# joncampbell123/composite-video-simulator

Hardware: AMD Instinct MI355X
Metric: frames/sec (output frames = fields; 720x486 NTSC, preset '-vhs'; steady-state pipelined throughput, 4 steps in flight) (higher is better)
Workload: dtype f64; 1 GPU; 720x486 30fps 10s colour-bars clip, preset '-vhs': 300 frames -> 600 fields per GPU per step, frame-round-robin over 1 GPU(s); steps_in_flight=4, mode=exact (bit-identical to the reference: fp64, no FMA contraction)

## Files before the change

composite-video-simulator_amd/csrc/ntsc_decode_fast.hip:

```cpp
#pragma clang fp contract(off)

namespace ntscsim {
namespace fastdec {

typedef uint32_t v4u __attribute__((ext_vector_type(4)));
#ifdef NTSC_PLAIN_OUT_STORES
#define NTSC_OUT_STORE(p, v) (*(p) = (v))
#else
#define NTSC_OUT_STORE(p, v) __builtin_nontemporal_store((v), (p))
#endif
typedef __attribute__((address_space(1))) v4u *g_v4u_ptr;
typedef __attribute__((address_space(1))) const v4u *g_cv4u_ptr;
DEV v4u to_v4u(const uint4 &a) { return v4u{a.x, a.y, a.z, a.w}; }
typedef __attribute__((address_space(1))) uint32_t *g_u32_ptr;
typedef __attribute__((address_space(1))) const uint32_t *g_cu32_ptr;

#ifdef NTSC_NO_STEP_SCHED_BARRIER
#define NTSC_STEP_SCHED_BARRIER() ((void)0)
#else
#define NTSC_STEP_SCHED_BARRIER() __builtin_amdgcn_sched_barrier(0)
#endif

struct LaneRand32 {
    uint32_t p3, p2, p1;
    int pos;
    DEV void init(uint32_t *ring, const uint32_t *state, int stride, int lane, int o)
    {
        for (int j = 0; j < 31; j++) {
            const uint32_t w = state[(size_t)j * stride];
            const int sl = (o + j) & 31;
            ring[sl * 64 + lane] = w;
            if (sl == 0) ring[32 * 64 + lane] = w;
            if (j == 28) p3 = w;
            if (j == 29) p2 = w;
            if (j == 30) p1 = w;
        }
        pos = (o + 31) & 31;
    }
    DEV uint32_t next(uint32_t *ring, int lane)
    {
        const uint32_t v = ring[(pos + 1) * 64 + lane] + p3;
        ring[pos * 64 + lane] = v;
        if (pos == 0) ring[32 * 64 + lane] = v;
        p3 = p2; p2 = p1; p1 = v;
        pos = (pos + 1) & 31;
        return v >> 1;
    }
    template <int K>
    DEV uint32_t draw(uint32_t *rb, bool first_slot_is_zero)
    {
        const uint32_t v = rb[(K + 1) * 64] + p3;
        rb[K * 64] = v;
        if (K == 0 && first_slot_is_zero) rb[32 * 64] = v;
        p3 = p2; p2 = p1; p1 = v;
        return v >> 1;
    }
};

template <class RT>
struct Casc3;
template <>
struct Casc3<double> {
    double r0, r1, r2;
    DEV void reset(double v, double a) { const double r = v - (v * a); r0 = r1 = r2 = r; }
    DEV double push(double s, double a, double &m2)
    {
        const double p0 = (s * a) + r0;
        const double m0 = p0 * a;
        r0 = p0 - m0;
        const double p1 = m0 + r1;
        const double m1 = p1 * a;
        r1 = p1 - m1;
        const double p2 = m1 + r2;
        m2 = p2 * a;
        r2 = p2 - m2;
        return p2;
    }
    DEV double push(double s, double a) { double m; return push(s, a, m); }
};
template <>
struct Casc3<float> {
    float p0, p1, p2;
    DEV void reset(float v, float) { p0 = p1 = p2 = v; }
    DEV float push(float s, float a, float &m2)
    {
        p0 = __builtin_fmaf(a, s - p0, p0);
        p1 = __builtin_fmaf(a, p0 - p1, p1);
        p2 = __builtin_fmaf(a, p1 - p2, p2);
        m2 = 0.f;
        return p2;
    }
    DEV float push(float s, float a) { float m; return push(s, a, m); }
};
template <class RT>
struct PoleHp;
template <>
struct PoleHp<double> {
    double r;
    DEV void reset(double v, double a) { r = v - (v * a); }
    DEV double hp(double s, double s_times_a, double a)
    {
        const double p = s_times_a + r;
        r = p - (p * a);
        return s - p;
    }
};
template <>
struct PoleHp<float> {
    float p;
    DEV void reset(float v, float) { p = v; }
    DEV float hp(float s, float, float a) { p = __builtin_fmaf(a, s - p, p); return s - p; }
};

DEV int sdiv4s(int n) { return (n + (int)((unsigned)n >> 30)) >> 2; }

DEV int scale_back50(int c, unsigned mul, unsigned shift)
{
    const int sg = c >> 31;
    const unsigned a = (unsigned)((c ^ sg) - sg) * 50u;
    const int q = (int)(__umulhi(a, mul) >> shift);
    return (q ^ sg) - sg;
}

struct DemodR {
    int c0, c1, c2, csum;
    int w0, w1, w2, w3, w4, w5;
    int y0, y1, y2, y3, y4;
    int ieP, qeP, ieN, qeN;
    DEV void init()
    {
        c0 = c1 = c2 = csum = 0;
        w0 = w1 = w2 = w3 = w4 = w5 = 0;
        y0 = y1 = y2 = y3 = y4 = 0;
        ieP = qeP = ieN = qeN = 0;
    }
    template <bool ODD, int NEG, bool LUMA, bool BK = false>
    DEV void push(int ct, bool hi, int sneg, int &Yo, int &Io, int &Qo, unsigned bmul = 0, unsigned bshift = 0)
    {
        const int yb = sdiv4s(csum + ct);
        int ch = ct - yb;
        if (BK) ch = scale_back50(ch, bmul, bshift);
        csum = csum - c0 + ct;
        c0 = c1; c1 = c2; c2 = ct;
        w0 = w1; w1 = w2; w2 = w3; w3 = w4; w4 = w5; w5 = ch;
        if (LUMA) { Yo = y0; y0 = y1; y1 = y2; y2 = y3; y3 = y4; y4 = yb; }
        if (ODD) {
            const int a = hi ? w3 : w1, b = hi ? w4 : w2;
            if (NEG == 0) { ieN = a; qeN = b; }
            else if (NEG == 1) { ieN = -a; qeN = -b; }
            else { ieN = (a ^ sneg) - sneg; qeN = (b ^ sneg) - sneg; }
            Io = (ieP + ieN) >> 1;
            Qo = (qeP + qeN) >> 1;
        } else {
            Io = ieN; Qo = qeN;
            ieP = ieN; qeP = qeN;
        }
    }
    template <bool BK = false, bool ANY = false>
    DEV void push_edge(int ct, int t, unsigned xi, bool hi, int W, int xe, int &Yo, int &Io, int &Qo,
                       unsigned bmul = 0, unsigned bshift = 0)
    {
        const int yb = sdiv4(c0 + c1 + c2 + ct);
        int ch = ct - yb;
        if (BK) ch = scale_back50(ch, bmul, bshift);
        csum = c1 + c2 + ct;
        c0 = c1; c1 = c2; c2 = ct;
        w0 = w1; w1 = w2; w2 = w3; w3 = w4; w4 = w5; w5 = ch;
        Yo = y0; y0 = y1; y1 = y2; y2 = y3; y3 = y4; y4 = yb;
        const int x = t - 7;
        int I, Q;
        if (x & 1) {
            const bool m = (x + 1 + (int)xi + 1) < W;
            const bool od = ANY && (xi & 1u) != 0;
            const int a = hi ? (od ? w4 : w3) : (od ? w2 : w1), b = hi ? (od ? w5 : w4) : (od ? w3 : w2);
            const bool pos = ANY ? ((((x + 1 + 2 * (int)xi) & 2) != 0) && !(xi == 1u && x == -1)) : ((x & 3) == 1);
            ieN = m ? (pos ? a : -a) : 0;
            qeN = m ? (pos ? b : -b) : 0;
            I = (ieP + ieN) >> 1;
            Q = (qeP + qeN) >> 1;
        } else {
            I = ieN; Q = qeN;
            ieP = ieN; qeP = qeN;
        }
        if (x >= xe) { I = 0; Q = 0; }
        Io = I; Qo = Q;
    }
};

struct DemodS {
    int c1, pA, pB;
    int e1, e2, o1, o2;
    int y0, y1, y2, y3, y4;
    int ieP, qeP, ieN, qeN;
    DEV void from(const DemodR &D, bool pick_next)
    {
        c1 = D.c2; pA = D.c2 + D.c1; pB = D.c1 + D.c0;
        if (pick_next) { e1 = D.w4; e2 = D.w2; o1 = D.w5; o2 = D.w3; }
        else           { e1 = D.w5; e2 = D.w3; o1 = D.w4; o2 = D.w2; }
        y0 = D.y0; y1 = D.y1; y2 = D.y2; y3 = D.y3; y4 = D.y4;
        ieP = D.ieP; qeP = D.qeP; ieN = D.ieN; qeN = D.qeN;
    }
    DEV void to(DemodR &D, bool pick_next) const
    {
        D.c2 = c1; D.c1 = pA - c1; D.c0 = pB - D.c1; D.csum = D.c0 + D.c1 + D.c2;
        D.w0 = 0; D.w1 = 0;
        if (pick_next) { D.w4 = e1; D.w2 = e2; D.w5 = o1; D.w3 = o2; }
        else           { D.w5 = e1; D.w3 = e2; D.w4 = o1; D.w2 = o2; }
        D.y0 = y0; D.y1 = y1; D.y2 = y2; D.y3 = y3; D.y4 = y4;
        D.ieP = ieP; D.qeP = qeP; D.ieN = ieN; D.qeN = qeN;
    }
    template <bool PICK, bool NEG, bool LUMA, bool BK = false, bool MASK = false, bool ANY = false>
    DEV void push(int ct, bool hi, int dm, int &Yo, int &Io, int &Qo, unsigned bmul = 0, unsigned bshift = 0,
                  bool odd = false, int mo = 0)
    {
        const int p = ct + c1;
        const int yb = sdiv4s(p + pB);
        int ch = ct - yb;
        if (BK) ch = scale_back50(ch, bmul, bshift);
        c1 = ct; pB = pA; pA = p;
        if (LUMA) { Yo = y0; y0 = y1; y1 = y2; y2 = y3; y3 = y4; y4 = yb; }
        if (PICK) {
            int a, b;
            if (ANY) {
                const int aL = odd ? o2 : e2, aH = odd ? o1 : e1;
                const int bL = odd ? e1 : o2, bH = odd ? ch : o1;
                a = hi ? aH : aL; b = hi ? bH : bL;
                const int sg = NEG ? ~mo : mo;
                a = (a ^ sg) - sg; b = (b ^ sg) - sg;
            } else {
                a = hi ? e1 : e2; b = hi ? o1 : o2;
                if (NEG) { a = -a; b = -b; }
            }
            e2 = e1; e1 = ch;
            if (MASK) { a &= dm; b &= dm; }
            ieN = a; qeN = b;
            Io = (ieP + ieN) >> 1;
            Qo = (qeP + qeN) >> 1;
        } else {
            o2 = o1; o1 = ch;
            Io = ieN; Qo = qeN;
            ieP = ieN; qeP = qeN;
        }
    }
};

template <bool VHS, class RT>
struct State {
    DemodR D1, D2;
    int l0, l1, l2, lsum;
    Casc3<RT> vl, vcU, vcV, sh, oU, oV;
    PoleHp<RT> vpre;
    int Yprev, Uraw, Vraw;
    RT Uf2[2];
    LaneRand32 rng;
    int nU, nV;
};

template <class RT, bool WR = false, bool BK = false, bool SV = false, bool XA = false, bool FO = false>
struct Const {
    static constexpr bool fullout = FO;
    static constexpr int SH = FO ? 3 : 0;
    RT a_oi, a_oq;
    uint32_t *xs;
    static constexpr bool wraps = WR;
    static constexpr bool back = BK;
    static constexpr bool svideo = SV;
    static constexpr bool anyxi = XA;
    bool odd;
    int mo;
    int ms[4];
    unsigned bmul, bshift;
    int wrapoff;
    int wrapA, wrapS;
    unsigned xi;
    bool hi;
    int W, xe, lane;
    int d, SKT, LOFF;
    int mL, mNL;
    int bA, bC;
    int dm;
    RT cosv, sinv;
    RT a_vc, a_vl, a_sh, a_tv, sharp2;
    int *tailU;
    size_t rstride;
    __amdgpu_buffer_rsrc_t comp;
    int vbase;
    int rowbytes;
};

#ifndef NTSC_COMP_LOAD2_AUX
#define NTSC_COMP_LOAD2_AUX 2
#endif
template <int AUX = 0, class CT>
DEV int cs_load(const CT &C, int x)
{
#ifdef NTSC_AB_NOLOAD
    return C.vbase + x;
#endif
    unsigned off = (unsigned)C.vbase + (unsigned)x * (unsigned)C.rowbytes;
    if constexpr (CT::wraps) off += (unsigned)((((C.wrapA - x) ^ C.wrapS) >> 31) & C.wrapoff);
    return __builtin_amdgcn_raw_buffer_load_b32(C.comp, (int)off, 0, AUX);
}

DEV int opaque_v(int v) { asm volatile("" : "+v"(v)); return v; }
DEV int opaque_s(int v) { return __builtin_amdgcn_readfirstlane(v); }

DEV int wave_up(int v) { return __builtin_amdgcn_update_dpp(0, v, 0x138, 0xf, 0xf, false); }

DEV uint32_t cvt_sat_u32(double x) { uint32_t r; asm("v_cvt_u32_f64 %0, %1" : "=v"(r) : "v"(x)); return r; }
DEV uint32_t cvt_sat_u32(float x) { uint32_t r; asm("v_cvt_u32_f32 %0, %1" : "=v"(r) : "v"(x)); return r; }
DEV uint32_t umin32(uint32_t a, uint32_t b) { return a < b ? a : b; }

template <class RT>
DEV uint32_t yiq_to_bgra(int Yo, RT fU, RT fV)
{
    const RT y = (RT)Yo;
#ifdef NTSC_OLD_CLAMP
    int r = (int)((y + (RT(0.956) * fU)) + (RT(0.621) * fV)) >> 8;
    int g = (int)((y + (RT(-0.272) * fU)) + (RT(-0.647) * fV)) >> 8;
    int b = (int)((y + (RT(-1.106) * fU)) + (RT(1.703) * fV)) >> 8;
    r = r < 0 ? 0 : (r > 255 ? 255 : r);
    g = g < 0 ? 0 : (g > 255 ? 255 : g);
    b = b < 0 ? 0 : (b > 255 ? 255 : b);
    return (((uint32_t)r << 16) | (uint32_t)b) | ((uint32_t)g << 8);
#else
    const uint32_t r = umin32(cvt_sat_u32((y + (RT(0.956) * fU)) + (RT(0.621) * fV)) >> 8, 255u);
    const uint32_t g = umin32(cvt_sat_u32((y + (RT(-0.272) * fU)) + (RT(-0.647) * fV)) >> 8, 255u);
    const uint32_t b = umin32(cvt_sat_u32((y + (RT(-1.106) * fU)) + (RT(1.703) * fV)) >> 8, 255u);
    return ((r << 16) | b) | (g << 8);
#endif
}

struct Steady {
    DemodS D1, D2;
    int lc1, lpA, lpB;
    uint32_t *rb;
    bool rb0;
    int yd[4];
    int ud[2];
};

template <int DPH, int J, class RT, class CT>
DEV int vcr_step(const DevParams &P, State<true, RT> &S, Steady &T, const CT &C,
                 int pc, int pl, int &Yv, int &Uv, int &Vv)
{
    constexpr bool pick1 = ((DPH + J) & 1) != 0;
    constexpr bool neg1 = ((DPH + J) & 3) == 3;
    int Yd, U, V;
    T.D1.template push<pick1, neg1, false, CT::back, false, CT::anyxi>(pc, C.hi, -1, Yd, U, V, C.bmul, C.bshift, C.odd, C.mo);
    U += S.nU; V += S.nV;
    S.nU = sdiv2(S.nU + (int)umod31(S.rng.template draw<2 * J>(T.rb, T.rb0), P.m_cnoise) - P.cnoise_k);
    S.nV = sdiv2(S.nV + (int)umod31(S.rng.template draw<2 * J + 1>(T.rb, T.rb0), P.m_cnoise) - P.cnoise_k);
    const RT u = (RT)U, v = (RT)V;
    const RT Ud = rtrunc<RT>((u * C.cosv) - (v * C.sinv));
    const RT Vd = rtrunc<RT>((u * C.sinv) + (v * C.cosv));
    const int fU = (int)S.vcU.push(Ud, C.a_vc);
    const int fV = (int)S.vcV.push(Vd, C.a_vc);
    const int lp = pl + T.lc1;
    const int yb = sdiv4s(lp + T.lpB);
    T.lc1 = pl; T.lpB = T.lpA; T.lpA = lp;
    RT m2;
    RT s = S.vl.push((RT)yb, C.a_vl, m2);
    s += S.vpre.hp(s, m2, C.a_vl) * RT(1.6);
    const RT s0 = rtrunc<RT>(s);
    const RT ts = S.sh.push(s0, C.a_sh);
    const int Y = (int)(s0 + ((s0 - ts) * C.sharp2));
    U = ((wave_up(fU) & C.bA) + fU + C.bC) >> C.bC;
    V = ((wave_up(fV) & C.bA) + fV + C.bC) >> C.bC;
    Yv = Y; Uv = U; Vv = V;
    constexpr int J2 = (J + CT::SH) & 3;
    if constexpr (CT::anyxi) {
        const int chroma = (J2 & 1) ? (C.odd ? U : V) : (C.odd ? V : U);
        const int mm = C.ms[J2];
        return Y + ((chroma ^ mm) - mm);
    }
    const int chroma = (J2 & 1) ? V : U;
    const int mm = (J2 & 2) ? C.mNL : C.mL;
    return Y + ((chroma ^ mm) - mm);
}

template <bool VHS, int DPH, int J, class RT, class CT>
DEV uint32_t step(const DevParams &P, State<VHS, RT> &S, Steady &T, const CT &C, int pc, int pl)
{
    int Y, U, V;
    constexpr bool pick3 = ((J + 1 + CT::SH) & 1) != 0;
    constexpr bool neg3 = ((J + 1 + CT::SH) & 3) == 3;
    if constexpr (!VHS) {
        T.D1.template push<pick3, neg3, true, CT::back, true, CT::anyxi>(pc, C.hi, C.dm, Y, U, V, C.bmul, C.bshift, C.odd, C.mo);
    } else {
        int Yv, Uv, Vv;
        const int c2 = vcr_step<DPH, J, RT, CT>(P, S, T, C, pc, pl, Yv, Uv, Vv);
        if constexpr (CT::svideo) {
            Y = Yv; U = Uv & C.dm; V = Vv & C.dm;
        } else {
            T.D2.template push<pick3, neg3, true, false, true, CT::anyxi>(c2, C.hi, C.dm, Y, U, V, 0, 0, C.odd, C.mo);
        }
    }
    if constexpr (CT::fullout) {
        const int fUn = (int)S.oU.push((RT)U, C.a_oi);
        const RT fVd = rtrunc<RT>(S.oV.push((RT)V, C.a_oq));
        const int Yo = T.yd[J];
        T.yd[J] = Y;
        const RT fUd = (RT)T.ud[J & 1];
        T.ud[J & 1] = fUn;
        return yiq_to_bgra<RT>(Yo, fUd, fVd);
    } else {
        const RT fUd = rtrunc<RT>(S.oU.push((RT)U, C.a_tv));
        const RT fVd = rtrunc<RT>(S.oV.push((RT)V, C.a_tv));
        const int Yo = S.Yprev;
        S.Yprev = Y;
        return yiq_to_bgra<RT>(Yo, fUd, fVd);
    }
}

template <class RT, class CT>
DEV int vcr_edge(const DevParams &P, State<true, RT> &S, const CT &C, uint32_t *ring, int t, int &Yv, int &Uv, int &Vv)
{
    const int W = C.W;
    const int pc = t < W ? cs_load(C, t) : 0;
    int Y, U, V;
    S.D1.template push_edge<CT::back, CT::anyxi>(pc, t, C.xi, C.hi, W, C.xe, Y, U, V, C.bmul, C.bshift);
    const int x1 = t - 7;
    const bool in1 = x1 >= 0 && x1 < W;
    int fU = 0, fV = 0;
    if (in1) {
        U += S.nU; V += S.nV;
        S.nU = sdiv2(S.nU + (int)umod31(S.rng.next(ring, C.lane), P.m_cnoise) - P.cnoise_k);
        S.nV = sdiv2(S.nV + (int)umod31(S.rng.next(ring, C.lane), P.m_cnoise) - P.cnoise_k);
        const RT u = (RT)U, v = (RT)V;
        U = (int)((u * C.cosv) - (v * C.sinv));
        V = (int)((u * C.sinv) + (v * C.cosv));
        fU = (int)S.vcU.push((RT)U, C.a_vc);
        fV = (int)S.vcV.push((RT)V, C.a_vc);
        if (x1 >= W - C.d) {
            C.tailU[(size_t)(x1 & 15) * C.rstride] = U;
            C.tailU[(size_t)(16 + (x1 & 15)) * C.rstride] = V;
        }
    }
    const int x2 = x1 - C.d;
    const int xl = t - C.LOFF;
    const int pl = (xl >= 0 && xl < W) ? cs_load(C, xl) : 0;
    const int yb = sdiv4(S.l0 + S.l1 + S.l2 + pl);
    S.lsum = S.l1 + S.l2 + pl;
    S.l0 = S.l1; S.l1 = S.l2; S.l2 = pl;
    const bool in2 = x2 >= 0 && x2 < W;
    if (in2) {
        if (x2 >= W - C.d) {
            fU = C.tailU[(size_t)(x2 & 15) * C.rstride];
            fV = C.tailU[(size_t)(16 + (x2 & 15)) * C.rstride];
        }
        RT m2;
        RT s = S.vl.push((RT)yb, C.a_vl, m2);
        s += S.vpre.hp(s, m2, C.a_vl) * RT(1.6);
        const RT s0 = rtrunc<RT>(s);
        const RT ts = S.sh.push(s0, C.a_sh);
        Y = (int)(s0 + ((s0 - ts) * C.sharp2));
    }
    U = ((wave_up(fU) & C.bA) + fU + C.bC) >> C.bC;
    V = ((wave_up(fV) & C.bA) + fV + C.bC) >> C.bC;
    int c2 = 0;
    Yv = 0; Uv = 0; Vv = 0;
    if (in2) {
        Yv = Y; Uv = U; Vv = V;
        const unsigned s = (C.xi + (unsigned)x2) & 3u;
        int chroma = (s & 1u) ? V : U;
        if (s & 2u) chroma = -chroma;
        c2 = Y + chroma;
    }
    return c2;
}

template <bool VHS, class RT, class CT>
DEV bool edge_step(const DevParams &P, State<VHS, RT> &S, const CT &C, uint32_t *ring, int t,
                   uint32_t &px, int &xo_out)
{
    const int W = C.W;
    int Y, U, V;
    int x3 = t - 7;
    if constexpr (VHS) {
        int Yv, Uv, Vv;
        const int c2 = vcr_edge<RT, CT>(P, S, C, ring, t, Yv, Uv, Vv);
        const int x2 = t - 7 - C.d;
        if constexpr (CT::svideo) {
            Y = Yv; U = Uv; V = Vv;
            x3 = x2;
        } else {
            S.D2.template push_edge<false, CT::anyxi>(c2, x2, C.xi, C.hi, W, C.xe, Y, U, V);
            x3 = x2 - 7;
        }
    } else {
        const int pc = t < W ? cs_load(C, t) : 0;
        S.D1.template push_edge<CT::back, CT::anyxi>(pc, t, C.xi, C.hi, W, C.xe, Y, U, V, C.bmul, C.bshift);
    }
    if constexpr (CT::fullout) {
        if (x3 < 0 || x3 >= W + 4) return false;
        const bool in3f = x3 < W;
        if (!in3f) { U = 0; V = 0; Y = 0; }
        U &= C.dm; V &= C.dm;
        RT fUn = 0, fVn = 0;
        if (in3f) {
            fUn = rtrunc<RT>(S.oU.push((RT)U, C.a_oi));
            fVn = rtrunc<RT>(S.oV.push((RT)V, C.a_oq));
        }
        const int k3 = x3 & 3;
        const int Yo4 = (int)C.xs[k3 * 64], Ur4 = (int)C.xs[(4 + k3) * 64], Vr4 = (int)C.xs[(8 + k3) * 64];
        C.xs[k3 * 64] = (uint32_t)Y; C.xs[(4 + k3) * 64] = (uint32_t)U; C.xs[(8 + k3) * 64] = (uint32_t)V;
        const RT Uf = S.Uf2[0];
        S.Uf2[0] = S.Uf2[1]; S.Uf2[1] = fUn;
        const int xof = x3 - 4;
        if (xof < 0) return false;
        const RT Uo = xof < W - 2 ? Uf : (RT)Ur4;
        const RT Vo = xof < W - 4 ? fVn : (RT)Vr4;
        px = yiq_to_bgra<RT>(Yo4, Uo, Vo);
        xo_out = xof;
        return true;
    }
    if (x3 < 0 || x3 > W) return false;
    const bool in3 = x3 < W;
    if (!in3) { U = 0; V = 0; Y = 0; }
    U &= C.dm; V &= C.dm;
    RT fUd = 0, fVd = 0;
    if (in3) {
        fUd = rtrunc<RT>(S.oU.push((RT)U, C.a_tv));
        fVd = rtrunc<RT>(S.oV.push((RT)V, C.a_tv));
    }
    const int xo = x3 - 1;
    const int Yo = S.Yprev;
    const int Ur = S.Uraw, Vr = S.Vraw;
    S.Yprev = Y; S.Uraw = U; S.Vraw = V;
    if (xo < 0) return false;
    if (xo >= W - 1) { fUd = (RT)Ur; fVd = (RT)Vr; }
    px = yiq_to_bgra<RT>(Yo, fUd, fVd);
    xo_out = xo;
    return true;
}

template <bool VHS, int DPH, class RT, class CT>
DEV int steady(const DevParams &P, State<VHS, RT> &S, const CT &C, uint32_t *ring, uint32_t *lring,
               uint32_t *ostage, const unsigned long long *orow, uint32_t *drow, bool is_out, int t)
{
    const int t_end = C.W - (C.d > 7 ? C.d - 7 : 0);
    const int SKT = C.SKT, LOFF = C.LOFF, lane = C.lane;
    if (t + 4 > t_end) return t;
    if (VHS && (S.rng.pos & 7)) return t;
    Steady T;
    constexpr bool pick3_next = ((1 + CT::SH) & 1) != 0;
    T.D1.from(S.D1, VHS ? (DPH & 1) != 0 : pick3_next);
    T.D2.from(S.D2, pick3_next);
    T.lc1 = S.l2; T.lpA = S.l2 + S.l1; T.lpB = S.l1 + S.l0;
    if constexpr (CT::fullout) {
#pragma unroll
        for (int q = 0; q < 4; q++) T.yd[q] = (int)C.xs[q * 64];
        T.ud[0] = (int)S.Uf2[0]; T.ud[1] = (int)S.Uf2[1];
    }
    DemodS &Dout = (VHS && !CT::svideo) ? T.D2 : T.D1;
    if (!(VHS && CT::svideo)) { Dout.ieP &= C.dm; Dout.qeP &= C.dm; Dout.ieN &= C.dm; Dout.qeN &= C.dm; }
    int sbase = VHS ? S.rng.pos : 0;
    constexpr int PD = 4;
    int pc[PD], pl[PD];
#pragma unroll
    for (int j = 0; j < PD; j++) { pc[j] = cs_load(C, t + j); pl[j] = VHS ? cs_load<NTSC_COMP_LOAD2_AUX>(C, t + j - LOFF) : 0; }
    constexpr bool PFTOP = !VHS;
    int pend_x = -1;
#ifdef NTSC_FAST_LANE_STORE
#define NTSC_FAST_FLUSH()                                                                         \
    if (pend_x >= 0) {                                                                            \
        if (is_out) {                                                                             \
            const uint4 *sp = reinterpret_cast<const uint4 *>(&ostage[lane * 20]);                \
            g_v4u_ptr dp = (g_v4u_ptr)(drow + pend_x);                                            \
            const uint4 a = sp[0], b = sp[1], c4 = sp[2], d4 = sp[3];                             \
            dp[0] = to_v4u(a); dp[1] = to_v4u(b); dp[2] = to_v4u(c4); dp[3] = to_v4u(d4);         \
        }                                                                                         \
        pend_x = -1;                                                                              \
    }
#else
#define NTSC_FAST_FLUSH()                                                                         \
    if (pend_x >= 0) {                                                                            \
        _Pragma("unroll")                                                                         \
        for (int k = 0; k < 4; k++) {                                                             \
            const int r = 16 * k + (lane >> 2);                                                   \
            const unsigned long long rp = orow[r];                                                \
            const uint4 v = *reinterpret_cast<const uint4 *>(&ostage[r * 20 + (lane & 3) * 4]);   \
            if (rp) NTSC_OUT_STORE((g_v4u_ptr)(rp + 4ull * (unsigned)(pend_x + (lane & 3) * 4)), to_v4u(v)); \
        }                                                                                         \
        pend_x = -1;                                                                              \
    }
#endif
#ifdef NTSC_FAST_STORE_AT_TOP
    constexpr bool FLUSH_TOP = true;
#else
    constexpr bool FLUSH_TOP = CT::wraps;
#endif
#ifndef NTSC_FAST_NO_ENTRY_WAIT
    __builtin_amdgcn_s_waitcnt(0x0F70);
#endif
    for (; t + 4 <= t_end; t += 4) {
        if constexpr (FLUSH_TOP) { NTSC_FAST_FLUSH() }
        uint32_t o[4];
        int nc[4] = {0, 0, 0, 0}, nl[4] = {0, 0, 0, 0};
        if (PFTOP) {
#pragma unroll
            for (int j = 0; j < 4; j++) { nc[j] = cs_load(C, t + 4 + j); nl[j] = VHS ? cs_load<NTSC_COMP_LOAD2_AUX>(C, t + 4 + j - LOFF) : 0; }
        }
        T.rb = ring + sbase * 64 + lane;
        T.rb0 = sbase == 0;
        sbase = (sbase + 8) & 31;
#define NTSC_FAST_STEP(J)                                                                         \
        o[J] = step<VHS, DPH, J, RT, CT>(P, S, T, C, pc[J % PD], pl[J % PD]);                     \
        if (!PFTOP) {                                                                             \
            pc[J % PD] = cs_load(C, t + PD + J);                                                  \
            if (VHS) pl[J % PD] = cs_load<NTSC_COMP_LOAD2_AUX>(C, t + PD + J - LOFF);                                  \
        }                                                                                         \
        NTSC_STEP_SCHED_BARRIER();
        NTSC_FAST_STEP(0)
        NTSC_FAST_STEP(1)
        NTSC_FAST_STEP(2)
        NTSC_FAST_STEP(3)
#undef NTSC_FAST_STEP
        if constexpr (PFTOP) {
#pragma unroll
            for (int j = 0; j < 4; j++) { pc[j] = nc[j]; pl[j] = nl[j]; }
        }
        const int xo0 = t - SKT;
        const int sub = (xo0 >> 2) & 3;
        *reinterpret_cast<uint4 *>(&ostage[lane * 20 + sub * 4]) = make_uint4(o[0], o[1], o[2], o[3]);
        if (sub == 3) pend_x = xo0 - 12;
        if constexpr (!FLUSH_TOP) { NTSC_FAST_FLUSH() }
    }
    NTSC_FAST_FLUSH()
#undef NTSC_FAST_FLUSH
    T.D1.to(S.D1, VHS ? (DPH & 1) != 0 : pick3_next);
    T.D2.to(S.D2, pick3_next);
    if constexpr (CT::fullout) {
#pragma unroll
        for (int q = 0; q < 4; q++) C.xs[q * 64] = (uint32_t)T.yd[q];
        S.Uf2[0] = (RT)T.ud[0]; S.Uf2[1] = (RT)T.ud[1];
    }
    S.Uraw = 0; S.Vraw = 0;
    S.l2 = T.lc1; S.l1 = T.lpA - T.lc1; S.l0 = T.lpB - S.l1; S.lsum = S.l0 + S.l1 + S.l2;
    if (VHS) S.rng.pos = sbase;
    return t;
}

}

#ifndef NTSC_FAST_WAVES
#define NTSC_FAST_WAVES 2
#endif
#ifndef NTSC_FAST_WAVES_F32
#define NTSC_FAST_WAVES_F32 2
#endif
template <class RT> struct FastWaves { static constexpr int n = NTSC_FAST_WAVES; };
template <> struct FastWaves<float> { static constexpr int n = NTSC_FAST_WAVES_F32; };
template <bool VHS, class RT, bool WR, bool BK, bool SV = false, bool XA = false, bool FO = false>
DEV void decode_fast_body(const DevParams &P, const GeomDev &G, const FieldDev *__restrict__ fields,
                          const int *__restrict__ comp, const uint32_t *__restrict__ rs_chroma,
                          const int *__restrict__ n0_u, const int *__restrict__ n0_v,
                          const int *__restrict__ hs_shift, const int *__restrict__ pn_noise,
                          const int *__restrict__ dropout, int *__restrict__ tails)
{
    using namespace fastdec;
    __shared__ uint32_t ring[33 * 64];
    __shared__ uint32_t lring[FO ? 12 * 64 : 64];
    __shared__ __attribute__((aligned(16))) uint32_t ostage[64 * 20];
    __shared__ unsigned long long orow[64];

    const int lane = threadIdx.x;
    const int gidx = blockIdx.x * 63 + lane - 1;
    const int rc = gidx < 0 ? 0 : (gidx < P.R ? gidx : P.R - 1);
    const int f = rc / P.Lslot, k = rc - f * P.Lslot;
    const FieldDev &fd = fields[f];
    const unsigned field = fd.field & 1u;
    const bool rowok = (int)(field + 2u * k) < P.H;
#ifdef NTSC_AB_NOSTORE
    const bool is_out = false;
#else
    const bool is_out = lane >= 1 && gidx < P.R && rowok;
#endif
    const unsigned y = rowok ? field + 2u * (unsigned)k : field;
    const int W = P.W;
    uint32_t *drow = reinterpret_cast<uint32_t *>(fd.dst + (size_t)fd.dst_ls * y);
    orow[lane] = is_out ? (unsigned long long)drow : 0ull;
    const size_t tcol = (size_t)blockIdx.x * 64 + lane;
    const size_t tstride = (size_t)gridDim.x * 64;

    typedef Const<RT, WR, BK, SV, XA, FO> CT;
    CT C;
    C.bmul = P.m_amp_back.mul; C.bshift = P.m_amp_back.shift;
    C.xi = scan_phase(P, y, fd.fieldno);
    C.hi = (C.xi & 2u) != 0;
    C.odd = (C.xi & 1u) != 0;
    if constexpr (XA) {
        C.mo = opaque_v(C.odd ? -1 : 0);
#pragma unroll
        for (int j = 0; j < 4; j++) C.ms[j] = opaque_v(((C.xi + (unsigned)j) & 2u) ? -1 : 0);
    }
    C.W = W;
    C.xe = (W & 1) ? W - 1 : W - 2;
    C.lane = lane;
    C.d = VHS ? P.cdelay : 0;
    C.SKT = (VHS ? (CT::svideo ? 8 : 15) + C.d : 8) + CT::SH;
    C.LOFF = 5 + C.d;
    C.mL = opaque_v(C.hi ? -1 : 0);
    C.mNL = opaque_v(~C.mL);
    const bool vb = VHS && P.vblend && P.ntsc;
    C.bA = opaque_v((vb && k >= 2) ? -1 : 0);
    C.bC = opaque_v((vb && k >= 1) ? 1 : 0);
    C.dm = opaque_v((P.loss && dropout[rc] != 0) ? 0 : -1);
    C.cosv = 1; C.sinv = 0;
    if (VHS) {
        int n = (rowok ? pn_noise[rc] : 0) + P.pnoise_k;
        n = n < 0 ? 0 : (n > 2 * P.pnoise_k ? 2 * P.pnoise_k : n);
        C.cosv = (RT)G.ptab[2 * n]; C.sinv = (RT)G.ptab[2 * n + 1];
    }
    C.a_vc = (RT)P.a_vc; C.a_vl = (RT)P.a_vl; C.a_sh = (RT)P.a_sh; C.a_tv = (RT)P.a_tv;
    C.a_oi = (RT)P.a_in_i; C.a_oq = (RT)P.a_in_q;
    C.sharp2 = (RT)(P.sharpen * 2);
    C.tailU = tails + tcol;
    C.rstride = tstride;
    C.rowbytes = P.Rpad * 4;
    const int hs = P.hs ? hs_shift[rc] : 0;
    C.vbase = (int)((unsigned)rc * 4u + (unsigned)hs * (unsigned)C.rowbytes);
    {
        const int tw = W + W / 10;
        C.wrapoff = (int)((unsigned)(hs > 0 ? -tw : tw) * (unsigned)C.rowbytes);
        C.wrapA = hs > 0 ? tw - hs - 1 : (hs < 0 ? -hs - 1 : 0x3FFFFFFF);
        C.wrapS = opaque_v(hs < 0 ? -1 : 0);
    }
    C.comp = __builtin_amdgcn_make_buffer_rsrc(const_cast<int *>(comp), 0,
                                               (int)((unsigned)W * (unsigned)C.rowbytes), 0x00020000);

    State<VHS, RT> S;
    S.D1.init(); S.D2.init();
    S.l0 = S.l1 = S.l2 = S.lsum = 0;
    S.vl.reset(16, C.a_vl); S.vpre.reset(16, C.a_vl); S.vcU.reset(0, C.a_vc); S.vcV.reset(0, C.a_vc);
    S.sh.reset(0, C.a_sh);
    if (CT::fullout) { S.oU.reset(0, C.a_oi); S.oV.reset(0, C.a_oq); }
    else { S.oU.reset(0, C.a_tv); S.oV.reset(0, C.a_tv); }
    S.Yprev = S.Uraw = S.Vraw = 0;
    C.xs = lring + lane;
    if (CT::fullout)
        for (int q = 0; q < 12; q++) C.xs[q * 64] = 0;
    S.Uf2[0] = S.Uf2[1] = 0;
    S.nU = S.nV = 0;
    if (VHS) {
        const int fill_draws = 2 * (C.SKT - 7);
        S.rng.init(ring, rs_chroma + rc, P.Rpad, lane, (-(31 + fill_draws)) & 7);
        S.nU = n0_u[rc]; S.nV = n0_v[rc];
    }

    const int SKT = C.SKT;
    const int total = W + SKT;
    int t = 0;
#ifdef NTSC_EDGE_UNROLL
#pragma unroll NTSC_EDGE_UNROLL
#endif
    for (; t < SKT && t < total; t++) {
        uint32_t px; int xo;
        (void)edge_step<VHS, RT, CT>(P, S, C, ring, t, px, xo);
    }
    if constexpr (!VHS) t = steady<VHS, 0, RT, CT>(P, S, C, ring, lring, ostage, orow, drow, is_out, t);
    else switch ((C.SKT - 7) & 3) {
        case 0: t = steady<VHS, 0, RT, CT>(P, S, C, ring, lring, ostage, orow, drow, is_out, t); break;
        case 1: t = steady<VHS, 1, RT, CT>(P, S, C, ring, lring, ostage, orow, drow, is_out, t); break;
        case 2: t = steady<VHS, 2, RT, CT>(P, S, C, ring, lring, ostage, orow, drow, is_out, t); break;
        default: t = steady<VHS, 3, RT, CT>(P, S, C, ring, lring, ostage, orow, drow, is_out, t); break;
    }
#ifdef NTSC_EDGE_UNROLL
#pragma unroll NTSC_EDGE_UNROLL
#endif
    for (; t < total; t++) {
        uint32_t px; int xo;
        if (!edge_step<VHS, RT, CT>(P, S, C, ring, t, px, xo)) continue;
        ostage[lane * 20 + (xo & 15)] = px;
        if ((xo & 15) == 15) {
            if (is_out) {
                const uint4 *sp = reinterpret_cast<const uint4 *>(&ostage[lane * 20]);
                g_v4u_ptr dp = (g_v4u_ptr)(drow + (xo - 15));
                const uint4 a = sp[0], b = sp[1], c4 = sp[2], d4 = sp[3];
                dp[0] = to_v4u(a); dp[1] = to_v4u(b); dp[2] = to_v4u(c4); dp[3] = to_v4u(d4);
            }
        } else if (xo == W - 1 && is_out) {
            const int xb = xo & ~15;
            for (int q = xb; q <= xo; q++) ((g_u32_ptr)drow)[q] = ostage[lane * 20 + (q - xb)];
        }
    }
}

template <bool VHS, class RT, bool WR = false>
__global__ __launch_bounds__(64, VHS ? FastWaves<RT>::n : 4) void k_decode_fast(DevParams P, GeomDev G,
                                                     const FieldDev *__restrict__ fields,
                                                     const int *__restrict__ comp,
                                                     const uint32_t *__restrict__ rs_chroma,
                                                     const int *__restrict__ n0_u,
                                                     const int *__restrict__ n0_v,
                                                     const int *__restrict__ hs_shift,
                                                     const int *__restrict__ pn_noise,
                                                     const int *__restrict__ dropout,
                                                     int *__restrict__ tails)
{
    decode_fast_body<VHS, RT, WR, false>(P, G, fields, comp, rs_chroma, n0_u, n0_v, hs_shift, pn_noise, dropout, tails);
}

template <bool VHS, class RT>
__global__ __launch_bounds__(64, VHS ? FastWaves<RT>::n : 4) void k_decode_fast_bk(DevParams P, GeomDev G,
                                                     const FieldDev *__restrict__ fields,
                                                     const int *__restrict__ comp,
                                                     const uint32_t *__restrict__ rs_chroma,
                                                     const int *__restrict__ n0_u,
                                                     const int *__restrict__ n0_v,
                                                     const int *__restrict__ hs_shift,
                                                     const int *__restrict__ pn_noise,
                                                     const int *__restrict__ dropout,
                                                     int *__restrict__ tails)
{
    decode_fast_body<VHS, RT, VHS, true>(P, G, fields, comp, rs_chroma, n0_u, n0_v, hs_shift, pn_noise, dropout, tails);
}

template <class RT>
__global__ __launch_bounds__(64, FastWaves<RT>::n) void k_decode_fast_xi(DevParams P, GeomDev G,
                                                     const FieldDev *__restrict__ fields,
                                                     const int *__restrict__ comp,
                                                     const uint32_t *__restrict__ rs_chroma,
                                                     const int *__restrict__ n0_u,
                                                     const int *__restrict__ n0_v,
                                                     const int *__restrict__ hs_shift,
                                                     const int *__restrict__ pn_noise,
                                                     const int *__restrict__ dropout,
                                                     int *__restrict__ tails)
{
    decode_fast_body<true, RT, true, false, false, true>(P, G, fields, comp, rs_chroma, n0_u, n0_v, hs_shift, pn_noise, dropout, tails);
}

template <class RT>
__global__ __launch_bounds__(64, FastWaves<RT>::n) void k_decode_fast_fo(DevParams P, GeomDev G,
                                                     const FieldDev *__restrict__ fields,
                                                     const int *__restrict__ comp,
                                                     const uint32_t *__restrict__ rs_chroma,
                                                     const int *__restrict__ n0_u,
                                                     const int *__restrict__ n0_v,
                                                     const int *__restrict__ hs_shift,
                                                     const int *__restrict__ pn_noise,
                                                     const int *__restrict__ dropout,
                                                     int *__restrict__ tails)
{
    decode_fast_body<true, RT, true, false, false, false, true>(P, G, fields, comp, rs_chroma, n0_u, n0_v, hs_shift, pn_noise, dropout, tails);
}

template <class RT>
__global__ __launch_bounds__(64, FastWaves<RT>::n) void k_decode_fast_sv(DevParams P, GeomDev G,
                                                     const FieldDev *__restrict__ fields,
                                                     const int *__restrict__ comp,
                                                     const uint32_t *__restrict__ rs_chroma,
                                                     const int *__restrict__ n0_u,
                                                     const int *__restrict__ n0_v,
                                                     const int *__restrict__ hs_shift,
                                                     const int *__restrict__ pn_noise,
                                                     const int *__restrict__ dropout,
                                                     int *__restrict__ tails)
{
    decode_fast_body<true, RT, true, false, true>(P, G, fields, comp, rs_chroma, n0_u, n0_v, hs_shift, pn_noise, dropout, tails);
}

#ifndef NTSC_FRONT_WAVES
#define NTSC_FRONT_WAVES 3
#endif
template <class RT>
__global__ __launch_bounds__(64, NTSC_FRONT_WAVES) void k_vcr_front(DevParams P, GeomDev G,
                                                      const FieldDev *__restrict__ fields,
                                                      const int *__restrict__ comp,
                                                      int *__restrict__ comp_out,
                                                      const uint32_t *__restrict__ rs_chroma,
                                                      const int *__restrict__ n0_u,
                                                      const int *__restrict__ n0_v,
                                                      const int *__restrict__ hs_shift,
                                                      const int *__restrict__ pn_noise,
                                                      int *__restrict__ tails)
{
    using namespace fastdec;
    __shared__ uint32_t ring[33 * 64];
    const int lane = threadIdx.x;
    const int gidx = blockIdx.x * 63 + lane - 1;
    const int rc = gidx < 0 ? 0 : (gidx < P.R ? gidx : P.R - 1);
    const int f = rc / P.Lslot, k = rc - f * P.Lslot;
    const FieldDev &fd = fields[f];
    const unsigned field = fd.field & 1u;
    const bool rowok = (int)(field + 2u * k) < P.H;
    const bool is_out = lane >= 1 && gidx < P.R;
    const unsigned y = rowok ? field + 2u * (unsigned)k : field;
    const int W = P.W;
    const size_t tcol = (size_t)blockIdx.x * 64 + lane;
    const size_t tstride = (size_t)gridDim.x * 64;

    typedef Const<RT, false> CT;
    CT C;
    C.wrapoff = 0; C.wrapA = 0x3FFFFFFF; C.wrapS = 0;
    C.xi = scan_phase(P, y, fd.fieldno);
    C.hi = (C.xi & 2u) != 0;
    C.W = W;
    C.xe = (W & 1) ? W - 1 : W - 2;
    C.lane = lane;
    C.d = P.cdelay;
    C.SKT = 7 + C.d;
    C.LOFF = 5 + C.d;
    C.mL = opaque_v(C.hi ? -1 : 0);
    C.mNL = opaque_v(~C.mL);
    const bool vb = P.vblend && P.ntsc;
    C.bA = opaque_v((vb && k >= 2) ? -1 : 0);
    C.bC = opaque_v((vb && k >= 1) ? 1 : 0);
    C.dm = -1;
    {
        int n = (rowok ? pn_noise[rc] : 0) + P.pnoise_k;
        n = n < 0 ? 0 : (n > 2 * P.pnoise_k ? 2 * P.pnoise_k : n);
        C.cosv = (RT)G.ptab[2 * n]; C.sinv = (RT)G.ptab[2 * n + 1];
    }
    C.a_vc = (RT)P.a_vc; C.a_vl = (RT)P.a_vl; C.a_sh = (RT)P.a_sh; C.a_tv = (RT)P.a_tv;
    C.sharp2 = (RT)(P.sharpen * 2);
    C.tailU = tails + tcol;
    C.rstride = tstride;
    C.rowbytes = P.Rpad * 4;
    const int hs = P.hs ? hs_shift[rc] : 0;
    C.vbase = (int)((unsigned)rc * 4u + (unsigned)hs * (unsigned)C.rowbytes);
    C.comp = __builtin_amdgcn_make_buffer_rsrc(const_cast<int *>(comp), 0,
                                               (int)((unsigned)W * (unsigned)C.rowbytes), 0x00020000);
    const __amdgpu_buffer_rsrc_t out = __builtin_amdgcn_make_buffer_rsrc(comp_out, 0,
                                               (int)((unsigned)W * (unsigned)C.rowbytes), 0x00020000);
    const int vout = (is_out ? gidx : P.R + lane) * 4;

    State<true, RT> S;
    S.D1.init(); S.D2.init();
    S.l0 = S.l1 = S.l2 = S.lsum = 0;
    S.vl.reset(16, C.a_vl); S.vpre.reset(16, C.a_vl); S.vcU.reset(0, C.a_vc); S.vcV.reset(0, C.a_vc);
    S.sh.reset(0, C.a_sh); S.oU.reset(0, C.a_tv); S.oV.reset(0, C.a_tv);
    S.Yprev = S.Uraw = S.Vraw = 0;
    S.rng.init(ring, rs_chroma + rc, P.Rpad, lane, (-(31 + 2 * (C.SKT - 7))) & 7);
    S.nU = n0_u[rc]; S.nV = n0_v[rc];

    const int SK1 = C.SKT, LOFF = C.LOFF;
    const int total = W + SK1;
    const unsigned rb = (unsigned)C.rowbytes;
    int t = 0;
    int yv_, uv_, vv_;
    for (; t < SK1 && t < total; t++) (void)vcr_edge<RT, CT>(P, S, C, ring, t, yv_, uv_, vv_);
    {
        const int t_end = W - (C.d > 7 ? C.d - 7 : 0);
        if (t + 4 <= t_end && !(S.rng.pos & 7)) {
            Steady T;
            T.D1.from(S.D1, (C.d & 1) != 0);
            T.D2.from(S.D2, true);
            T.lc1 = S.l2; T.lpA = S.l2 + S.l1; T.lpB = S.l1 + S.l0;
            int sbase = S.rng.pos;
            int pc[4], pl[4];
#pragma unroll
            for (int j = 0; j < 4; j++) { pc[j] = cs_load(C, t + j); pl[j] = cs_load<NTSC_COMP_LOAD2_AUX>(C, t + j - LOFF); }
            unsigned soff = (unsigned)(t - SK1) * rb;
#define NTSC_VCR_STEP(DPV, J)                                                                     \
            {                                                                                     \
                const int c2 = vcr_step<DPV, J, RT, CT>(P, S, T, C, pc[J], pl[J], yv_, uv_, vv_); \
                pc[J] = cs_load(C, t + 4 + J);         \
                pl[J] = cs_load<NTSC_COMP_LOAD2_AUX>(C, t + 4 + J - LOFF);                                             \
                __builtin_amdgcn_raw_buffer_store_b32(c2, out, vout, (int)soff, 0);               \
                soff += rb;                                                                       \
                NTSC_STEP_SCHED_BARRIER();                                                        \
            }
#define NTSC_VCR_ITER(DPV)                                                                        \
            for (; t + 4 <= t_end; t += 4) {                                                      \
                T.rb = ring + sbase * 64 + lane; T.rb0 = sbase == 0; sbase = (sbase + 8) & 31;    \
                NTSC_VCR_STEP(DPV, 0) NTSC_VCR_STEP(DPV, 1) NTSC_VCR_STEP(DPV, 2) NTSC_VCR_STEP(DPV, 3)  \
            }
            switch (C.d & 3) {
                case 0: NTSC_VCR_ITER(0) break;
                case 1: NTSC_VCR_ITER(1) break;
                case 2: NTSC_VCR_ITER(2) break;
                default: NTSC_VCR_ITER(3) break;
            }
#undef NTSC_VCR_ITER
#undef NTSC_VCR_STEP
            T.D1.to(S.D1, (C.d & 1) != 0);
            S.l2 = T.lc1; S.l1 = T.lpA - T.lc1; S.l0 = T.lpB - S.l1; S.lsum = S.l0 + S.l1 + S.l2;
            S.rng.pos = sbase;
        }
    }
    for (; t < total; t++) {
        const int c2 = vcr_edge<RT, CT>(P, S, C, ring, t, yv_, uv_, vv_);
        const int x2 = t - SK1;
        if (x2 >= 0) __builtin_amdgcn_raw_buffer_store_b32(c2, out, vout, (int)((unsigned)x2 * rb), 0);
    }
}

}
```

Measured before the change: 811,100 frames/s.

## Prefetch RNG ring words ahead and reschedule input reloads and output flush

Hoists the LDS reads of the lagged-Fibonacci RNG ring words one step ahead of their use in the VHS steady loop, so the draws no longer wait on a dependent LDS load. Input composite sample reloads are delayed by one step (LATE), with opaque_v barriers pinning the chains. The output flush is split into batched row-pointer and staging loads, then a waitcnt, then the stores. This reshapes instruction scheduling to hide LDS and global latency, at the cost of extra registers and possible occupancy pressure.

New measurement: 817,700 frames/s (median of 6 runs). About the same (+0.8%).

```diff
diff --git a/composite-video-simulator_amd/csrc/ntsc_decode_fast.hip b/composite-video-simulator_amd/csrc/ntsc_decode_fast.hip
--- a/composite-video-simulator_amd/csrc/ntsc_decode_fast.hip
+++ b/composite-video-simulator_amd/csrc/ntsc_decode_fast.hip
@@ -47,14 +47,16 @@
         return v >> 1;
     }
     template <int K>
-    DEV uint32_t draw(uint32_t *rb, bool first_slot_is_zero)
-    {
-        const uint32_t v = rb[(K + 1) * 64] + p3;
+    DEV uint32_t draw(uint32_t *rb, bool first_slot_is_zero, uint32_t w31)
+    {
+        const uint32_t v = w31 + p3;
         rb[K * 64] = v;
         if (K == 0 && first_slot_is_zero) rb[32 * 64] = v;
         p3 = p2; p2 = p1; p1 = v;
         return v >> 1;
     }
+    template <int K>
+    DEV uint32_t draw(uint32_t *rb, bool first_slot_is_zero) { return draw<K>(rb, first_slot_is_zero, rb[(K + 1) * 64]); }
 };
 
 template <class RT>
@@ -336,6 +338,8 @@
     int lc1, lpA, lpB;
     uint32_t *rb;
     bool rb0;
+    uint32_t rw[4][2];
+    template <int J> DEV void ring_words(const uint32_t *b) { rw[J][0] = b[(2 * J + 1) * 64]; rw[J][1] = b[(2 * J + 2) * 64]; }
     int yd[4];
     int ud[2];
 };
@@ -348,9 +352,12 @@
     constexpr bool neg1 = ((DPH + J) & 3) == 3;
     int Yd, U, V;
     T.D1.template push<pick1, neg1, false, CT::back, false, CT::anyxi>(pc, C.hi, -1, Yd, U, V, C.bmul, C.bshift, C.odd, C.mo);
+#ifndef NTSC_AB_RELOAD_AT_STEP
+    if (pick1) T.D1.e1 = opaque_v(T.D1.e1); else T.D1.o1 = opaque_v(T.D1.o1);
+#endif
     U += S.nU; V += S.nV;
-    S.nU = sdiv2(S.nU + (int)umod31(S.rng.template draw<2 * J>(T.rb, T.rb0), P.m_cnoise) - P.cnoise_k);
-    S.nV = sdiv2(S.nV + (int)umod31(S.rng.template draw<2 * J + 1>(T.rb, T.rb0), P.m_cnoise) - P.cnoise_k);
+    S.nU = sdiv2(S.nU + (int)umod31(S.rng.template draw<2 * J>(T.rb, T.rb0, T.rw[J][0]), P.m_cnoise) - P.cnoise_k);
+    S.nV = sdiv2(S.nV + (int)umod31(S.rng.template draw<2 * J + 1>(T.rb, T.rb0, T.rw[J][1]), P.m_cnoise) - P.cnoise_k);
     const RT u = (RT)U, v = (RT)V;
     const RT Ud = rtrunc<RT>((u * C.cosv) - (v * C.sinv));
     const RT Vd = rtrunc<RT>((u * C.sinv) + (v * C.cosv));
@@ -389,7 +396,10 @@
         T.D1.template push<pick3, neg3, true, CT::back, true, CT::anyxi>(pc, C.hi, C.dm, Y, U, V, C.bmul, C.bshift, C.odd, C.mo);
     } else {
         int Yv, Uv, Vv;
-        const int c2 = vcr_step<DPH, J, RT, CT>(P, S, T, C, pc, pl, Yv, Uv, Vv);
+        int c2 = vcr_step<DPH, J, RT, CT>(P, S, T, C, pc, pl, Yv, Uv, Vv);
+#ifndef NTSC_AB_RELOAD_AT_STEP
+        c2 = opaque_v(c2);
+#endif
         if constexpr (CT::svideo) {
             Y = Yv; U = Uv & C.dm; V = Vv & C.dm;
         } else {
@@ -558,8 +568,16 @@
     int sbase = VHS ? S.rng.pos : 0;
     constexpr int PD = 4;
     int pc[PD], pl[PD];
+#ifdef NTSC_AB_RELOAD_AT_STEP
+    constexpr bool LATE = false;
+#else
+    constexpr bool LATE = VHS;
+#endif
 #pragma unroll
-    for (int j = 0; j < PD; j++) { pc[j] = cs_load(C, t + j); pl[j] = VHS ? cs_load<NTSC_COMP_LOAD2_AUX>(C, t + j - LOFF) : 0; }
+    for (int j = 0; j < PD; j++) {
+        if (LATE && j == PD - 1) { pc[j] = 0; pl[j] = 0; continue; }
+        pc[j] = cs_load(C, t + j); pl[j] = VHS ? cs_load<NTSC_COMP_LOAD2_AUX>(C, t + j - LOFF) : 0;
+    }
     constexpr bool PFTOP = !VHS;
     int pend_x = -1;
 #ifdef NTSC_FAST_LANE_STORE
@@ -574,15 +592,28 @@
         pend_x = -1;                                                                              \
     }
 #else
+#ifdef NTSC_AB_FLUSH_CHAIN
+#define NTSC_FLUSH_PIN() ((void)0)
+#define NTSC_FLUSH_WAIT() ((void)0)
+#else
+#define NTSC_FLUSH_PIN() __builtin_amdgcn_sched_barrier(0)
+#define NTSC_FLUSH_WAIT() __builtin_amdgcn_s_waitcnt(0xC07F)
+#endif
 #define NTSC_FAST_FLUSH()                                                                         \
     if (pend_x >= 0) {                                                                            \
+        unsigned long long rp[4];                                                                 \
+        uint4 v[4];                                                                               \
+        NTSC_FLUSH_PIN();                                                                         \
         _Pragma("unroll")                                                                         \
-        for (int k = 0; k < 4; k++) {                                                             \
-            const int r = 16 * k + (lane >> 2);                                                   \
-            const unsigned long long rp = orow[r];                                                \
-            const uint4 v = *reinterpret_cast<const uint4 *>(&ostage[r * 20 + (lane & 3) * 4]);   \
-            if (rp) NTSC_OUT_STORE((g_v4u_ptr)(rp + 4ull * (unsigned)(pend_x + (lane & 3) * 4)), to_v4u(v)); \
-        }                                                                                         \
+        for (int k = 0; k < 4; k++) rp[k] = orow[16 * k + (lane >> 2)];                           \
+        _Pragma("unroll")                                                                         \
+        for (int k = 0; k < 4; k++)                                                               \
+            v[k] = *reinterpret_cast<const uint4 *>(&ostage[(16 * k + (lane >> 2)) * 20 + (lane & 3) * 4]); \
+        NTSC_FLUSH_WAIT();                                                                        \
+        NTSC_FLUSH_PIN();                                                                         \
+        _Pragma("unroll")                                                                         \
+        for (int k = 0; k < 4; k++)                                                               \
+            if (rp[k]) NTSC_OUT_STORE((g_v4u_ptr)(rp[k] + 4ull * (unsigned)(pend_x + (lane & 3) * 4)), to_v4u(v[k])); \
         pend_x = -1;                                                                              \
     }
 #endif
@@ -594,6 +625,12 @@
 #ifndef NTSC_FAST_NO_ENTRY_WAIT
     __builtin_amdgcn_s_waitcnt(0x0F70);
 #endif
+#ifdef NTSC_AB_RING_AT_DRAW
+    constexpr bool RING_AHEAD = false;
+#else
+    constexpr bool RING_AHEAD = true;
+#endif
+    if (VHS && RING_AHEAD) T.template ring_words<0>(ring + sbase * 64 + lane);
     for (; t + 4 <= t_end; t += 4) {
         if constexpr (FLUSH_TOP) { NTSC_FAST_FLUSH() }
         uint32_t o[4];
@@ -605,13 +642,29 @@
         T.rb = ring + sbase * 64 + lane;
         T.rb0 = sbase == 0;
         sbase = (sbase + 8) & 31;
+        const uint32_t *rbn = ring + sbase * 64 + lane;
 #define NTSC_FAST_STEP(J)                                                                         \
-        o[J] = step<VHS, DPH, J, RT, CT>(P, S, T, C, pc[J % PD], pl[J % PD]);                     \
-        if (!PFTOP) {                                                                             \
-            pc[J % PD] = cs_load(C, t + PD + J);                                                  \
-            if (VHS) pl[J % PD] = cs_load<NTSC_COMP_LOAD2_AUX>(C, t + PD + J - LOFF);                                  \
-        }                                                                                         \
-        NTSC_STEP_SCHED_BARRIER();
+        {                                                                                         \
+            if (VHS && !RING_AHEAD) T.template ring_words<J>(T.rb);                               \
+            if (VHS && RING_AHEAD && J < 3) {                                                     \
+                if (J == 0) { T.template ring_words<1>(T.rb); T.template ring_words<2>(T.rb); }   \
+                if (J == 1) T.template ring_words<3>(T.rb);                                       \
+                if (J == 2) T.template ring_words<0>(rbn);                                        \
+                NTSC_STEP_SCHED_BARRIER();                                                        \
+            }                                                                                     \
+            o[J] = step<VHS, DPH, J, RT, CT>(P, S, T, C, pc[J % PD], pl[J % PD]);                 \
+            if (!PFTOP && !LATE) {                                                                \
+                pc[J % PD] = cs_load(C, t + PD + J);                                              \
+                if (VHS) pl[J % PD] = cs_load<NTSC_COMP_LOAD2_AUX>(C, t + PD + J - LOFF);         \
+            }                                                                                     \
+            if (!PFTOP && LATE) {                                                                 \
+                constexpr int Jr = (J + PD - 1) % PD;                                             \
+                const int tr = t + Jr + (J == 0 ? 0 : PD);                                        \
+                pc[Jr] = cs_load(C, tr);                                                          \
+                pl[Jr] = cs_load<NTSC_COMP_LOAD2_AUX>(C, tr - LOFF);                              \
+            }                                                                                     \
+            NTSC_STEP_SCHED_BARRIER();                                                            \
+        }
         NTSC_FAST_STEP(0)
         NTSC_FAST_STEP(1)
         NTSC_FAST_STEP(2)
@@ -629,6 +682,14 @@
     }
     NTSC_FAST_FLUSH()
 #undef NTSC_FAST_FLUSH
+#undef NTSC_FLUSH_PIN
+#undef NTSC_FLUSH_WAIT
+#ifndef NTSC_AB_RELOAD_AT_STEP
+    if (LATE) {
+        T.D1.pA = opaque_v(T.D1.pA); T.D1.pB = opaque_v(T.D1.pB);
+        T.lpA = opaque_v(T.lpA); T.lpB = opaque_v(T.lpB);
+    }
+#endif
     T.D1.to(S.D1, VHS ? (DPH & 1) != 0 : pick3_next);
     T.D2.to(S.D2, pick3_next);
     if constexpr (CT::fullout) {
@@ -956,6 +1017,7 @@
             unsigned soff = (unsigned)(t - SK1) * rb;
 #define NTSC_VCR_STEP(DPV, J)                                                                     \
             {                                                                                     \
+                T.template ring_words<J>(T.rb);                                                   \
                 const int c2 = vcr_step<DPV, J, RT, CT>(P, S, T, C, pc[J], pl[J], yv_, uv_, vv_); \
                 pc[J] = cs_load(C, t + 4 + J);         \
                 pl[J] = cs_load<NTSC_COMP_LOAD2_AUX>(C, t + 4 + J - LOFF);                                             \
```
